# CristianSimion5/vk-raytracing-engine

Measured on AMD Instinct MI355X. Metric: Mrays/s, higher is better.
Workload: dtype f32

## Files before the change

vk-raytracing-engine_amd/csrc/shade.h:

```cpp
#pragma once
#include "device_math.h"
#include "device_scene.h"
#include "traverse.h"

struct Payload
{
  f3 hitValue;
  uint32_t seed;
  uint32_t depth;
  f3 rayOrigin, rayDirection, weight;
  bool isSpecular;
  float lightDist;
  f3 shadowRayDir;
};

struct ShadeStats
{
  unsigned hits, diffuse, taps;
  const float* lut;
};

VKRT_DEV const float* ldsTexelLut(const DevScene& sc, float* lds512)
{
  for(unsigned i = threadIdx.x; i < 512u; i += blockDim.x)
// ... 277 lines not shown
{
  f3 worldPos, N, tangent, binormal, V, baseColor, emittance;
  float metalU, roughU;
  unsigned retap;
};

VKRT_DEV void closestHitFront(const DevScene& sc, const RayHit& hit, const uint32_t instId, const uint4 ts, f3 worldRayDir, const Payload& prd,
                              ShadeStats& st, HitMid& mid)
{
  st.hits++;
  const uint32_t i0 = ts.x, i1 = ts.y, i2 = ts.z, matIndex = ts.w;
  const f3 b = mk3(1.0f - hit.u - hit.v, hit.u, hit.v);

  const BufView vPN = bufView(sc.vertexPN), vMat = bufView(sc.shadeMaterials), vInst = bufView(sc.instances);
  const float4 a0 = bufLoad4(vPN, VKRT_VERTEX_BYTES * i0), b0 = bufLoad4(vPN, VKRT_VERTEX_BYTES * i0 + 16u), tq0 = bufLoad4(vPN, VKRT_VERTEX_BYTES * i0 + 32u);
  const float4 a1 = bufLoad4(vPN, VKRT_VERTEX_BYTES * i1), b1 = bufLoad4(vPN, VKRT_VERTEX_BYTES * i1 + 16u), tq1 = bufLoad4(vPN, VKRT_VERTEX_BYTES * i1 + 32u);
  const float4 a2 = bufLoad4(vPN, VKRT_VERTEX_BYTES * i2), b2 = bufLoad4(vPN, VKRT_VERTEX_BYTES * i2 + 16u), tq2 = bufLoad4(vPN, VKRT_VERTEX_BYTES * i2 + 32u);
  const uint32_t mo = 64u * matIndex;
  const float4 m0 = bufLoad4(vMat, mo), m1 = bufLoad4(vMat, mo + 16u), ref01 = bufLoad4(vMat, mo + 32u), ref23 = bufLoad4(vMat, mo + 48u);
  const uint32_t dimB = __float_as_uint(ref01.x), baseB = __float_as_uint(ref01.y), dimM = __float_as_uint(ref01.z), baseM = __float_as_uint(ref01.w);
  const uint32_t dimN = __float_as_uint(ref23.x), baseN = __float_as_uint(ref23.y), dimE = __float_as_uint(ref23.z), baseE = __float_as_uint(ref23.w);
  DevInstance in;
  {
    const uint32_t io = 96u * instId;
    const float4 q0 = bufLoad4(vInst, io), q1 = bufLoad4(vInst, io + 16u), q2 = bufLoad4(vInst, io + 32u), q3 = bufLoad4(vInst, io + 48u), q4 = bufLoad4(vInst, io + 64u),
                 q5 = bufLoad4(vInst, io + 80u);
    in.o2w[0] = q0.x; in.o2w[1] = q0.y; in.o2w[2] = q0.z; in.o2w[3] = q0.w; in.o2w[4] = q1.x; in.o2w[5] = q1.y; in.o2w[6] = q1.z; in.o2w[7] = q1.w;
    in.o2w[8] = q2.x; in.o2w[9] = q2.y; in.o2w[10] = q2.z; in.o2w[11] = q2.w;
    in.w2o[0] = q3.x; in.w2o[1] = q3.y; in.w2o[2] = q3.z; in.w2o[3] = q3.w; in.w2o[4] = q4.x; in.w2o[5] = q4.y; in.w2o[6] = q4.z; in.w2o[7] = q4.w;
    in.w2o[8] = q5.x; in.primMesh = __float_as_int(q5.y); in.vis = 0u; in.pad = 0;
  }
  GltfPBRMaterial mat;
  mat.pbrBaseColorFactor[0] = m0.x; mat.pbrBaseColorFactor[1] = m0.y; mat.pbrBaseColorFactor[2] = m0.z; mat.pbrBaseColorFactor[3] = 1.0f;
  mat.metallicFactor = m0.w; mat.roughnessFactor = m1.x;
  mat.emissiveFactor[0] = m1.y; mat.emissiveFactor[1] = m1.z; mat.emissiveFactor[2] = m1.w;
  mat.pbrBaseColorTexture = (dimB & 0x8000u) ? 0 : -1; mat.metallicRoughnessTexture = (dimM & 0x8000u) ? 0 : -1;
  mat.normalTexture = (dimN & 0x8000u) ? 0 : -1; mat.emissiveTexture = (dimE & 0x8000u) ? 0 : -1;
  const float tu = (b0.z * b.x + b1.z * b.y) + b2.z * b.z;
  const float tv = (b0.w * b.x + b1.w * b.y) + b2.w * b.z;

  const bool emits = prd.depth == 0 || prd.isSpecular;
  const bool wantE = emits && mat.emissiveTexture > -1, wantN = mat.normalTexture > -1;
  const bool wantB = mat.pbrBaseColorTexture > -1, wantM = mat.metallicRoughnessTexture > -1;
  st.taps += (wantE ? 1u : 0u) + (wantN ? 1u : 0u) + (wantB ? 1u : 0u) + (wantM ? 1u : 0u);
  TexTap tE, tN, tB, tM;
#define VKRT_FOOTPRINT(dim, base, want, tap)                                                                                           \
  texFootprint(sc.texQuads ? 0u : ((base) & 0x7fffffffu), ((dim) & 0x7fffu) + 1u, (((dim) >> 16) & 0x7fffu) + 1u, ((base) >> 31) != 0u, \
               ((dim) >> 31) != 0u, want, tu, tv, tap)
  VKRT_FOOTPRINT(dimE, baseE, wantE, tE);
  VKRT_FOOTPRINT(dimN, baseN, wantN, tN);
  VKRT_FOOTPRINT(dimB, baseB, wantB, tB);
  VKRT_FOOTPRINT(dimM, baseM, wantM, tM);
#undef VKRT_FOOTPRINT
  uint32_t e00, e10, e01, e11, n00, n10, n01, n11, c00, c10, c01, c11, r00, r10, r01, r11;
  if(sc.texQuads)
  {
    const BufView quads = bufView(sc.texQuads);
#define VKRT_QUAD(dim, base, tap, want, a, b, c, d)                                                                                    \
  {                                                                                                                                    \
    const uint32_t rec_ = ((want) && ((dim) >> 31) != 0u) ? tap.i00 + ((base) & 0x7fffffffu) : 0u;                                        \
    const float4 v_ = bufLoad4(quads, 16u * rec_);                                                                                     \
    a = __float_as_uint(v_.x); b = __float_as_uint(v_.y); c = __float_as_uint(v_.z); d = __float_as_uint(v_.w);                        \
  }
    VKRT_QUAD(dimE, baseE, tE, wantE, e00, e10, e01, e11)
    VKRT_QUAD(dimN, baseN, tN, wantN, n00, n10, n01, n11)
    VKRT_QUAD(dimB, baseB, tB, wantB, c00, c10, c01, c11)
    VKRT_QUAD(dimM, baseM, tM, wantM, r00, r10, r01, r11)
#undef VKRT_QUAD
  }
  else
  {
    const BufView tex = bufView(sc.texels);
#define VKRT_TEXEL(i) bufLoad1(tex, 4u * (i))
    e00 = VKRT_TEXEL(tE.i00); e10 = VKRT_TEXEL(tE.i10); e01 = VKRT_TEXEL(tE.i01); e11 = VKRT_TEXEL(tE.i11);
    n00 = VKRT_TEXEL(tN.i00); n10 = VKRT_TEXEL(tN.i10); n01 = VKRT_TEXEL(tN.i01); n11 = VKRT_TEXEL(tN.i11);
    c00 = VKRT_TEXEL(tB.i00); c10 = VKRT_TEXEL(tB.i10); c01 = VKRT_TEXEL(tB.i01); c11 = VKRT_TEXEL(tB.i11);
    r00 = VKRT_TEXEL(tM.i00); r10 = VKRT_TEXEL(tM.i10); r01 = VKRT_TEXEL(tM.i01); r11 = VKRT_TEXEL(tM.i11);
#undef VKRT_TEXEL
  }

  const f3 pos = mk3(a0.x, a0.y, a0.z) * b.x + mk3(a1.x, a1.y, a1.z) * b.y + mk3(a2.x, a2.y, a2.z) * b.z;
  const f3 worldPos = xformPoint(in, pos);
  const f3 nrm = normalize3(mk3(a0.w, b0.x, b0.y) * b.x + mk3(a1.w, b1.x, b1.y) * b.y + mk3(a2.w, b2.x, b2.y) * b.z);
  const f3 worldNrm = normalize3(xformNormal(in, nrm));
  const f3 tag = normalize3(mk3(tq0.x, tq0.y, tq0.z) * b.x + mk3(tq1.x, tq1.y, tq1.z) * b.y + mk3(tq2.x, tq2.y, tq2.z) * b.z);
  f3 worldTag = normalize3(xformNormal(in, tag));
  worldTag = normalize3(worldTag - dot3(worldTag, worldNrm) * worldNrm);
  const f3 worldBin = tq0.w * cross3(worldNrm, worldTag);

  f3 emittance = mk3(0.0f);
  if(emits)
  {
    emittance = mk3(mat.emissiveFactor[0], mat.emissiveFactor[1], mat.emissiveFactor[2]);
    if(wantE)
    {
      const f4 t = texBlend(st.lut, tE, e00, e10, e01, e11);
      emittance = emittance * mk3(t.x, t.y, t.z);
    }
  }
  f3 tangent = worldTag, binormal = worldBin;
  f3 texNormal = worldNrm;
  if(wantN)
  {
    const f4 t = texBlend(st.lut, tN, n00, n10, n01, n11);
    texNormal = normalize3(mk3(t.x, t.y, t.z) * 2.0f - mk3(1.0f));
    texNormal = normalize3(tangent * texNormal.x + binormal * texNormal.y + worldNrm * texNormal.z);
    createCoordinateSystem(texNormal, tangent, binormal);
  }
  f3 baseColor = mk3(mat.pbrBaseColorFactor[0], mat.pbrBaseColorFactor[1], mat.pbrBaseColorFactor[2]);
  if(wantB)
  {
    const f4 t = texBlend(st.lut, tB, c00, c10, c01, c11);
    baseColor = baseColor * mk3(t.x, t.y, t.z);
  }
  float metalness = mat.metallicFactor, roughness = mat.roughnessFactor;
  if(wantM)
  {
    const f4 t = texBlend(st.lut, tM, r00, r10, r01, r11);
    roughness *= t.y;
    metalness *= t.z;
  }

  mid.worldPos = worldPos; mid.N = texNormal; mid.tangent = tangent; mid.binormal = binormal;
  mid.V = normalize3(-worldRayDir);
  mid.baseColor = baseColor; mid.emittance = emittance;
  mid.metalU = metalness; mid.roughU = roughness;
  mid.retap = (mat.pbrBaseColorTexture > -1 ? 1u : 0u) + (mat.metallicRoughnessTexture > -1 ? 1u : 0u);
}

VKRT_DEV bool closestHitLobe(const HitMid& mid, Payload& prd)
// ... 105 lines not shown
```

vk-raytracing-engine_amd/csrc/wavefront.hip:

```cpp
#include <hip/hip_runtime.h>
#include <algorithm>
#include <cstdlib>
#include <cstring>

#include "device_math.h"
#include "device_scene.h"
#include "kernels.h"
#include "rgen.h"
#include "shade.h"
#include "traverse.h"
#include "traverse_wide.h"
#include "traverse_share.h"

#define WF_BLOCK 256
#define VKRT_FLAG_COUNT_WORK 2u

#include "wf_streams.h"

VKRT_DEV unsigned packFlags(const LaneState& L)
{
  return (L.prd.depth & 0xffu) | (((unsigned)L.smpl & 0xffffu) << 8) | ((L.prd.isSpecular ? 1u : 0u) << 25);
}

VKRT_DEV void loadCommon(const TraceParams& P, const WfBuffers& B, int parity, int type, unsigned i, LaneState& L)
{
  const float4 s0 = wfLoad(rec(B, parity, type, WF_S0, i)), s1 = wfLoad(rec(B, parity, type, WF_S1, i)), s2 = wfLoad(rec(B, parity, type, WF_S2, i));
  const unsigned flags = __float_as_uint(s1.w), pix = __float_as_uint(s2.w);
  L.curWeight = mk3(s0.x, s0.y, s0.z); L.prd.seed = __float_as_uint(s0.w);
  L.hitValue = mk3(s1.x, s1.y, s1.z);
  L.prd.depth = flags & 0xffu; L.smpl = (int)((flags >> 8) & 0xffffu);
  L.prd.isSpecular = ((flags >> 25) & 1u) != 0u;
  L.hitValues = mk3(s2.x, s2.y, s2.z);
  L.px = pix & 0xffffu; L.lrow = pix >> 16;
  float origin[4];
  mat4MulVec4(P.viewInverse, 0.0f, 0.0f, 0.0f, 1.0f, origin);
  L.camOrigin = mk3(origin[0], origin[1], origin[2]);
  L.prd.lightDist = 0.0f;
  L.prd.shadowRayDir = mk3(0.0f);
  L.prd.hitValue = mk3(0.0f);
  L.prd.weight = mk3(0.0f);
  L.stage = 0;
}

VKRT_DEV void storeState(const WfBuffers& B, int parity, int type, unsigned i, const LaneState& L, f3 weight)
{
  wfStore(rec(B, parity, type, WF_S0, i), make_float4(weight.x, weight.y, weight.z, __uint_as_float(L.prd.seed)));
  wfStore(rec(B, parity, type, WF_S1, i), make_float4(L.hitValue.x, L.hitValue.y, L.hitValue.z, __uint_as_float(packFlags(L))));
  wfStore(rec(B, parity, type, WF_S2, i), make_float4(L.hitValues.x, L.hitValues.y, L.hitValues.z, __uint_as_float(L.px | (L.lrow << 16))));
}

VKRT_DEV void storeClosest(const WfBuffers& B, int parity, unsigned i, const LaneState& L)
{
  wfStore(rec(B, parity, WF_C, WF_R0, i), make_float4(L.prd.rayOrigin.x, L.prd.rayOrigin.y, L.prd.rayOrigin.z, 10000.0f));
  wfStore(rec(B, parity, WF_C, WF_R1, i), make_float4(L.prd.rayDirection.x, L.prd.rayDirection.y, L.prd.rayDirection.z, 0.0f));
  storeState(B, parity, WF_C, i, L, L.curWeight);
}

VKRT_DEV void storeShadow(const WfBuffers& B, int parity, int type, unsigned i, const LaneState& L, f3 contrib, f3 nextWeight)
{
  wfStore(rec(B, parity, type, WF_R0, i), make_float4(L.prd.rayOrigin.x, L.prd.rayOrigin.y, L.prd.rayOrigin.z, L.prd.lightDist - 0.1f));
  wfStore(rec(B, parity, type, WF_R1, i), make_float4(L.prd.shadowRayDir.x, L.prd.shadowRayDir.y, L.prd.shadowRayDir.z, L.prd.lightDist));
  if(type == WF_P)
    wfStore(rec(B, parity, type, WF_R2, i), make_float4(L.prd.rayDirection.x, L.prd.rayDirection.y, L.prd.rayDirection.z, 0.0f));
  storeState(B, parity, type, i, L, nextWeight);
  wfStore(rec(B, parity, type, WF_S3, i), make_float4(contrib.x, contrib.y, contrib.z, 0.0f));
}

VKRT_DEV unsigned claimSlots(const WfBuffers& B, int parity, int to, unsigned lane, unsigned* wsum)
{
  const unsigned wave = threadIdx.x >> 6, nw = blockDim.x >> 6;
  const unsigned long long m[WF_TYPES] = {__ballot(to == WF_C), __ballot(to == WF_S), __ballot(to == WF_P)};
  if(lane == 0)
  {
#pragma unroll
    for(int t = 0; t < WF_TYPES; t++) wsum[t * (nw + 1) + wave] = (unsigned)__popcll(m[t]);
  }
  __syncthreads();
  if(threadIdx.x < WF_TYPES)
  {
    unsigned* w = wsum + threadIdx.x * (nw + 1);
    unsigned tot = 0;
    for(unsigned k = 0; k < nw; k++)
    {
      const unsigned c = w[k];
      w[k] = tot;
      tot += c;
    }
    w[nw] = tot ? atomicAdd(countOf(B, parity, (int)threadIdx.x), tot) : 0u;
  }
  __syncthreads();
  if(to < 0)
    return 0u;
  const unsigned long long below = (1ull << lane) - 1ull;
  const unsigned long long mine = to == WF_C ? m[0] : to == WF_S ? m[1] : m[2];
  return wsum[to * (nw + 1) + nw] + wsum[to * (nw + 1) + wave] + (unsigned)__popcll(mine & below);
}

__global__ __launch_bounds__(WF_BLOCK) void k_wf_init(const TraceParams P, const WfBuffers B)
{
  const unsigned lane = lane_id();
  const unsigned w = blockIdx.x * blockDim.x + threadIdx.x;
  bool alive = false;
  unsigned nPixels = 0;
  LaneState L;
  if(w < P.tileCount * 64u)
  {
    const unsigned tile = P.tileFirst + (w >> 6), inTile = w & 63u;
    const uint32_t x = (tile % P.tilesX) * 8u + (inTile & 7u);
    const uint32_t lrow = (tile / P.tilesX) * 8u + (inTile >> 3);
    if(x < P.fullW && lrow < P.localRows)
    {
      const uint32_t y = globalRow(P, lrow);
      if(y < P.fullH)
      {
        startPixel(P, L, x, y, lrow);
        nPixels = 1;
        if(P.pc.samples <= 0 || P.pc.depth <= 0)
          storePixel(P, L);
        else
          alive = true;
      }
    }
  }
  __shared__ unsigned wsum[WF_TYPES * (WF_BLOCK / 64 + 1)];
  const unsigned slot = claimSlots(B, 0, alive ? WF_C : -1, lane, wsum);
  if(alive)
    storeClosest(B, 0, slot, L);
  __shared__ unsigned long long red[VKRT_COUNTER_STRIDE * (WF_BLOCK / 64)];
  const unsigned vals[6] = {0, 0, 0, 0, 0, nPixels};
  blockAddCounters(&P.counters->v[blockIdx.x % VKRT_COUNTER_SLOTS][0], vals, 6, red);
}

VKRT_DEV void hybridFinish(const TraceParams& P, const HybridGi& G, uint32_t px, uint32_t lrow, bool shaded, f3 hitValue, float hitDists, float alpha)
{
  const size_t p = (size_t)lrow * P.fullW + px;
  float4 color = make_float4(0.0f, 0.0f, 0.0f, alpha);
  if(shaded)
  {
    color.x = hitValue.x; color.y = hitValue.y; color.z = hitValue.z;
    if(G.nrdRadHitD)
    {
      const float roughness = G.rough[p].x;
      const float viewZ = G.nrdViewZ[p];
      const float t = glsl_clamp(exp2f(-25.0f * roughness * roughness), 0.0f, 1.0f);
      const float f = (3.0f + fabsf(viewZ) * 1.0f) * (1.0f * (1.0f - t) + 20.0f * t);
      float normHitDist = glsl_clamp(hitDists / f, 0.0f, 1.0f);
      f3 rad = hitValue;
      const bool bad = isnan(rad.x) || isnan(rad.y) || isnan(rad.z) || isinf(rad.x) || isinf(rad.y) || isinf(rad.z);
      rad = bad ? mk3(0.0f) : mk3(glsl_clamp(rad.x, 0.0f, 65504.0f), glsl_clamp(rad.y, 0.0f, 65504.0f), glsl_clamp(rad.z, 0.0f, 65504.0f));
      normHitDist = (isnan(normHitDist) || isinf(normHitDist)) ? 0.0f : glsl_clamp(normHitDist, 0.0f, 1.0f);
      if(normHitDist != 0.0f)
        normHitDist = glsl_max(normHitDist, 1e-7f);
      const float Y = (rad.x * 0.25f + rad.y * 0.5f) + rad.z * 0.25f;
      const float Co = (rad.x * 0.5f + rad.y * 0.0f) + rad.z * -0.5f;
      const float Cg = (rad.x * -0.25f + rad.y * 0.5f) + rad.z * -0.25f;
      G.nrdRadHitD[p] = make_float4(quantizeHalf(Y), quantizeHalf(Co), quantizeHalf(Cg), quantizeHalf(normHitDist));
    }
  }
  if(P.pc.frame > 0)
  {
    const float a = 1.0f / (float)(P.pc.frame + 1);
    const float4 old = G.accum[p];
    G.accum[p] = make_float4(old.x * (1.0f - a) + color.x * a, old.y * (1.0f - a) + color.y * a, old.z * (1.0f - a) + color.z * a,
                             old.w * (1.0f - a) + color.w * a);
  }
  else
    G.accum[p] = color;
}
VKRT_DEV bool advanceSegmentHybrid(const TraceParams& P, const HybridGi& G, LaneState& L, bool shadowHit, f3 contrib, f3 nextWeight, float lightDist)
{
  L.stage = 0;
  if(!shadowHit)
    L.hitValue = L.hitValue + contrib;
  if(L.prd.depth == 1u && !L.prd.isSpecular)
    L.hitValues.x = shadowHit ? 0.5f * lightDist : lightDist;
  L.curWeight = nextWeight;
  L.prd.depth++;
  if(!(L.prd.depth < (uint32_t)P.pc.depth))
  {
    hybridFinish(P, G, L.px, L.lrow, true, L.hitValue, L.hitValues.x, L.hitValues.y);
    return false;
  }
  return true;
}

struct ShadeLds
{
  float lut[512];
  unsigned wsum[WF_TYPES * (WF_BLOCK / 64 + 1)];
};

template <bool PAIR, bool HYBRID>
VKRT_DEV void shadeHitBlock(const TraceParams& P, const WfBuffers& B, const HybridGi& G, const int par, const unsigned count, const unsigned block, ShadeLds& lds)
{
  const int type = PAIR ? WF_P : WF_C;
  const unsigned lane = lane_id();
  const unsigned qi = block * WF_BLOCK + threadIdx.x;
  ShadeStats st;
  st.hits = 0; st.diffuse = 0; st.taps = 0;
  st.lut = ldsTexelLut(P.sc, lds.lut);
  unsigned* wsum = lds.wsum;
  int to = -1;
  LaneState L;
  f3 contrib = mk3(0.0f), nextWeight = mk3(0.0f);
  if(qi < count)
  {
    loadCommon(P, B, par, type, qi, L);
    const float4 h = wfLoad(rec(B, par, type, WF_H0, qi)), t4 = wfLoad(rec(B, par, type, WF_H1, qi));
    const float4 rd = wfLoad(rec(B, par, type, PAIR ? WF_R2 : WF_R1, qi));
    L.prd.rayDirection = mk3(rd.x, rd.y, rd.z);
    L.prd.rayOrigin = mk3(0.0f);
    if(PAIR)
    {
      const float4 s3 = wfLoad(rec(B, par, WF_P, WF_S3, qi));
      const bool shadowHit = __float_as_int(h.x) != 0;
      if(HYBRID)
        (void)advanceSegmentHybrid(P, G, L, shadowHit, mk3(s3.x, s3.y, s3.z), L.curWeight, L.prd.depth == 1u ? wfLoad(rec(B, par, WF_P, WF_R1, qi)).w : 0.0f);
      else
        (void)advanceSegment(P, L, shadowHit, mk3(s3.x, s3.y, s3.z), L.curWeight);
    }
    RayHit hit;
    hit.t = h.x; hit.u = h.y; hit.v = h.z; hit.slot = __float_as_int(h.w);
    const uint4 ts = make_uint4(__float_as_uint(t4.x), __float_as_uint(t4.y), __float_as_uint(t4.z), __float_as_uint(t4.w));
    if(hit.slot >= 0)
      closestHitShaderInst(P.sc, P.pc, hit, (uint32_t)hit.slot, ts, L.prd.rayDirection, L.prd, st);
    else
      missShader(P.pc, L.prd);
    segmentTerms(L, contrib, nextWeight);
    const bool dead = !HYBRID && (P.flags & VKRT_FLAG_SKIP_DEAD_SHADOW) != 0u && contrib.x == 0.0f && contrib.y == 0.0f && contrib.z == 0.0f;
    if(!L.prd.isSpecular && L.prd.depth != 100u && !dead)
      to = (L.prd.depth + 1u < (uint32_t)P.pc.depth) ? WF_P : WF_S;
    else if(HYBRID)
      to = advanceSegmentHybrid(P, G, L, false, contrib, nextWeight, 0.0f) ? WF_C : -1;
    else
      to = advanceSegment(P, L, false, contrib, nextWeight) ? WF_C : -1;
  }
  const unsigned slot = claimSlots(B, par ^ 1, to, lane, wsum);
  if(to == WF_C)
    storeClosest(B, par ^ 1, slot, L);
  else if(to >= 0)
    storeShadow(B, par ^ 1, to, slot, L, contrib, nextWeight);
  if(P.flags & VKRT_FLAG_COUNT_WORK)
  {
    __shared__ unsigned long long red[VKRT_COUNTER_STRIDE * (WF_BLOCK / 64)];
    const unsigned vals[5] = {0, 0, st.hits, st.diffuse, st.taps};
    blockAddCounters(&P.counters->v[blockIdx.x % VKRT_COUNTER_SLOTS][0], vals, 5, red);
  }
}

template <bool HYBRID>
VKRT_DEV void shadeShadowBlock(const TraceParams& P, const WfBuffers& B, const HybridGi& G, const int par, const unsigned count, const unsigned block, ShadeLds& lds)
{
  const unsigned lane = lane_id();
  const unsigned qi = block * WF_BLOCK + threadIdx.x;
  unsigned* wsum = lds.wsum;
  bool toClosest = false;
  LaneState L;
  if(qi < count)
  {
    loadCommon(P, B, par, WF_S, qi, L);
    const float4 h = wfLoad(rec(B, par, WF_S, WF_H0, qi)), s3 = wfLoad(rec(B, par, WF_S, WF_S3, qi));
    L.prd.rayOrigin = mk3(0.0f);
    L.prd.rayDirection = mk3(0.0f);
    const bool shadowHit = __float_as_int(h.w) >= 0;
    if(HYBRID)
      toClosest = advanceSegmentHybrid(P, G, L, shadowHit, mk3(s3.x, s3.y, s3.z), L.curWeight, L.prd.depth == 1u ? wfLoad(rec(B, par, WF_S, WF_R1, qi)).w : 0.0f);
    else
      toClosest = advanceSegment(P, L, shadowHit, mk3(s3.x, s3.y, s3.z), L.curWeight);
  }
  const unsigned slot = claimSlots(B, par ^ 1, toClosest ? WF_C : -1, lane, wsum);
  if(toClosest)
    storeClosest(B, par ^ 1, slot, L);
}

template <bool HYBRID>
VKRT_DEV void shadeRound(const TraceParams& P, const WfBuffers& B, const HybridGi& G, const int round)
{
  const int par = round & 1;
  const unsigned cC = *countOf(B, par, WF_C), cS = *countOf(B, par, WF_S), cP = *countOf(B, par, WF_P);
  const unsigned nC = (cC + WF_BLOCK - 1) / WF_BLOCK, nP = (cP + WF_BLOCK - 1) / WF_BLOCK, nS = (cS + WF_BLOCK - 1) / WF_BLOCK;
  unsigned blk = blockIdx.x;
  __shared__ ShadeLds lds;
  if(blk < nC)
    shadeHitBlock<false, HYBRID>(P, B, G, par, cC, blk, lds);
  else if((blk -= nC) < nP)
    shadeHitBlock<true, HYBRID>(P, B, G, par, cP, blk, lds);
  else if((blk -= nP) < nS)
    shadeShadowBlock<HYBRID>(P, B, G, par, cS, blk, lds);
}
__global__ __launch_bounds__(WF_BLOCK) void k_wf_shade(const TraceParams P, const WfBuffers B, const int round)
{
  const HybridGi none{};
  shadeRound<false>(P, B, none, round);
}
__global__ __launch_bounds__(WF_BLOCK) void k_wf_shade_hybrid(const TraceParams P, const WfBuffers B, const HybridGi G, const int round)
{
  shadeRound<true>(P, B, G, round);
}

__global__ __launch_bounds__(WF_BLOCK) void k_hy_gi_init(const TraceParams P, const WfBuffers B, const HybridGi G, const uint2* tmp)
{
  const unsigned lane = lane_id();
  const unsigned w = blockIdx.x * blockDim.x + threadIdx.x;
  bool alive = false;
  LaneState L;
  if(w < P.tileCount * 64u)
  {
    const unsigned tile = P.tileFirst + (w >> 6), inTile = w & 63u;
    const uint32_t x = (tile % P.tilesX) * 8u + (inTile & 7u);
    const uint32_t lrow = (tile / P.tilesX) * 8u + (inTile >> 3);
    if(x < P.fullW && lrow < P.localRows && globalRow(P, lrow) < P.fullH)
    {
      const size_t p = (size_t)lrow * P.fullW + x;
      const float4 pixelImg = G.color[p], pixelPos = G.position[p], pixelNorm = G.normal[p];
      const float2 rm = G.rough[p];
      const uint2 t = tmp[p];
      const f3 worldPos = mk3(pixelPos.x, pixelPos.y, pixelPos.z), worldNrm = mk3(pixelNorm.x, pixelNorm.y, pixelNorm.z);
      const bool shaded = !(worldPos.x == 0.0f && worldPos.y == 0.0f && worldPos.z == 0.0f && worldNrm.x == 0.0f && worldNrm.y == 0.0f &&
                            worldNrm.z == 0.0f);
      const float alpha = __uint_as_float(t.y);
      if(!shaded)
        hybridFinish(P, G, x, lrow, false, mk3(0.0f), 0.0f, alpha);
      else
      {
        L.px = x; L.lrow = lrow;
        L.prd.seed = t.x;
        L.prd.lightDist = 0.0f; L.prd.shadowRayDir = mk3(0.0f);
        const float roughness = rm.x, metalness = rm.y;
        const float ratio = metalness * (1.0f - roughness);
        f3 direction;
        if(ratio < 0.8f)
        {
          L.prd.isSpecular = false;
          f3 tangent, binormal;
          createCoordinateSystem(worldNrm, tangent, binormal);
          direction = normalize3(samplingHemisphere(L.prd.seed, tangent, binormal, worldNrm));
          L.curWeight = mk3(pixelImg.w, pixelPos.w, pixelNorm.w);
        }
        else
        {
          L.prd.isSpecular = true;
          float cam[4];
          mat4MulVec4(P.viewInverse, 0.0f, 0.0f, 0.0f, 1.0f, cam);
          const f3 V = normalize3(mk3(cam[0], cam[1], cam[2]) - worldPos);
          direction = normalize3(glsl_reflect(-V, worldNrm));
          L.curWeight = mk3(1.0f);
        }
        L.prd.hitValue = mk3(0.0f);
        L.prd.rayOrigin = worldPos;
        L.prd.rayDirection = direction;
        L.prd.depth = 1;
        L.prd.weight = mk3(0.0f);
        L.hitValue = mk3(0.0f);
        L.hitValues = mk3(0.0f, alpha, 0.0f);
        L.smpl = 0;
        L.stage = 0;
        if(L.prd.depth < (uint32_t)P.pc.depth)
          alive = true;
        else
          hybridFinish(P, G, x, lrow, true, mk3(0.0f), 0.0f, alpha);
      }
    }
  }
  __shared__ unsigned wsum[WF_TYPES * (WF_BLOCK / 64 + 1)];
  const unsigned slot = claimSlots(B, 0, alive ? WF_C : -1, lane, wsum);
  if(alive)
    storeClosest(B, 0, slot, L);
}

__global__ __launch_bounds__(WF_BLOCK) void k_wf_blend(const TraceParams P, const float4* stage)
{
  const unsigned w = blockIdx.x * blockDim.x + threadIdx.x;
  if(w >= P.tileCount * 64u)
    return;
  const unsigned tile = P.tileFirst + (w >> 6), inTile = w & 63u;
  const uint32_t x = (tile % P.tilesX) * 8u + (inTile & 7u);
  const uint32_t lrow = (tile / P.tilesX) * 8u + (inTile >> 3);
  if(x < P.fullW && lrow < P.localRows && globalRow(P, lrow) < P.fullH)
  {
    const size_t p = (size_t)lrow * P.fullW + x;
    blendPixel((float4*)P.image + p, stage[p], P.pc.frame);
  }
}

#define WF_CTRL_BYTES (256 * VKRT_WF_MAX_LANES)
size_t vkrt_wf_state_bytes(uint32_t pathCapacity, int groups)
{
  const size_t g = (size_t)std::max(groups, 1);
  return g * pathCapacity * 2 * WF_SLOTS * sizeof(float4) + (g > 1 ? g * pathCapacity * sizeof(float4) : 0) + WF_CTRL_BYTES;
}

void vkrt_wf_carve(void* base, uint32_t pathCapacity, int groups, WfBuffers* B)
{
  const size_t g = (size_t)std::max(groups, 1);
  char* p = (char*)base;
  B->ctrl = (unsigned*)p;
  p += WF_CTRL_BYTES;
  B->planes = (float4*)p;
  p += g * pathCapacity * 2 * WF_SLOTS * sizeof(float4);
  B->stage = g > 1 ? (float4*)p : nullptr;
  B->capacity = pathCapacity;
  B->groups = (uint32_t)g;
}

static hipError_t subframeBegin(const TraceParams& P, const WfBuffers& B, hipStream_t stream)
{
  const unsigned work = P.tileCount * 64u;
  const hipError_t e = hipMemsetAsync(B.ctrl, 0, 64, stream);
  if(e != hipSuccess)
    return e;
  hipLaunchKernelGGL(k_wf_init, dim3((work + WF_BLOCK - 1) / WF_BLOCK), dim3(WF_BLOCK), 0, stream, P, B);
  return hipSuccess;
}
static int subframeRounds(const TraceParams& P) { return (P.pc.samples <= 0 || P.pc.depth <= 0) ? 0 : P.pc.samples * (P.pc.depth + 1); }
static void subframeRound(const TraceParams& P, const WfBuffers& B, int r, unsigned travBlock, bool count, hipStream_t stream, WfTiming* timing)
{
  const unsigned work = P.tileCount * 64u;
  const dim3 tg(2 * ((work + travBlock - 1) / travBlock) + 4);
  const size_t tlds = (size_t)P.sc.stackCap * travBlock * sizeof(int);
  const bool timed = timing && timing->events && 2 * (timing->used + 1) <= timing->capacity;
  if(timed)
    (void)hipEventRecord(timing->events[2 * timing->used], stream);
  vkrt_wf_launch_traverse(P, B, r, travBlock, count, tg, tlds, stream);
  if(timed)
  {
    (void)hipEventRecord(timing->events[2 * timing->used + 1], stream);
    timing->used++;
  }
  hipLaunchKernelGGL(k_wf_shade, dim3((work + WF_BLOCK - 1) / WF_BLOCK + 3), dim3(WF_BLOCK), 0, stream, P, B, r);
}

static TraceParams frameParams(const TraceParams& P, int k, uint32_t seedStep)
{
  TraceParams Q = P;
  Q.pc.frame = P.pc.frame + k;
  Q.seed = P.seed + (uint32_t)k * seedStep;
  return Q;
}

static int balancedInFlight(int frames, int want)
{
  want = std::max(1, std::min(want, frames));
  const int turns = (frames + want - 1) / want;
  return (frames + turns - 1) / turns;
}

hipError_t vkrt_launch_wavefront(const TraceParams& P, const WfBuffers& B, const WfOptions& opt, int frames, uint32_t seedStep, bool count,
                                 hipStream_t stream, WfTiming* timing, const WfAsync* async)
{
  const unsigned travBlock = opt.travBlock == 256 ? 256u : opt.travBlock == 128 ? 128u : 64u;
  const int rounds = subframeRounds(P);
  frames = std::max(frames, 1);
  int F = (timing || !async || rounds == 0) ? 1 : std::min(balancedInFlight(frames, opt.inFlight), (int)B.groups);
  F = std::max(1, std::min(F, async ? std::min(VKRT_WF_MAX_LANES, async->count) : 1));
  int S = (timing || !async || F > 1) ? 1 : std::max(1, std::min(std::min(VKRT_WF_MAX_LANES, opt.subframes), async->count));
  S = (int)std::min<uint32_t>((uint32_t)S, std::max(1u, P.tileCount / 256u));
  const int L = S * F;
  hipError_t e;
  if(L <= 1)
  {
    for(int k = 0; k < frames; k++)
    {
      TraceParams Q = frameParams(P, k, seedStep);
      Q.tileFirst = 0;
      if((e = subframeBegin(Q, B, stream)) != hipSuccess) return e;
      for(int r = 0; r < rounds; r++) subframeRound(Q, B, r, travBlock, count, stream, timing);
    }
    return hipGetLastError();
  }
  const bool staged = F > 1;
  if(staged && vkrt_wf_pool_events(frames, S) > async->poolSize)
    return hipErrorInvalidValue;
  hipStream_t laneStream[VKRT_WF_MAX_LANES];
  uint32_t tile0[VKRT_WF_MAX_LANES], tileN[VKRT_WF_MAX_LANES];
  WfBuffers Bq[VKRT_WF_MAX_LANES];
  const size_t groupQuads = (size_t)2 * WF_SLOTS * B.capacity;
  for(int q = 0; q < L; q++)
  {
    const int g = q / S, j = q % S;
    tile0[q] = (uint32_t)((uint64_t)P.tileCount * j / S);
    tileN[q] = (uint32_t)((uint64_t)P.tileCount * (j + 1) / S) - tile0[q];
    Bq[q].ctrl = B.ctrl + 64 * q;
    Bq[q].planes = B.planes + (size_t)g * groupQuads + (size_t)2 * WF_SLOTS * ((size_t)tile0[q] * 64u);
    Bq[q].stage = staged ? B.stage + (size_t)g * B.capacity : nullptr;
    Bq[q].capacity = tileN[q] * 64u;
    Bq[q].groups = 1;
    laneStream[q] = async->streams[q];
  }
  int forked = 0;
  auto joinLanes = [&]() {
    hipError_t first = hipSuccess;
    for(int q = 0; q < forked; q++)
    {
      hipError_t x = hipEventRecord(async->join[q], laneStream[q]);
      if(x == hipSuccess) x = hipStreamWaitEvent(stream, async->join[q], 0);
      if(x != hipSuccess)
      {
        (void)hipStreamSynchronize(laneStream[q]);
        if(first == hipSuccess) first = x;
      }
    }
    return first;
  };
  if((e = hipEventRecord(async->fork, stream)) != hipSuccess) return e;
  for(int q = 0; q < L; q++)
  {
    if((e = hipStreamWaitEvent(laneStream[q], async->fork, 0)) != hipSuccess)
    {
      (void)joinLanes();
      return e;
    }
    forked = q + 1;
  }
  const int items = rounds + 1 + (staged ? 1 : 0);
  hipEvent_t* evBlend = async->pool;
  int laneFrames[VKRT_WF_MAX_LANES], cursor[VKRT_WF_MAX_LANES];
  std::vector<char> blendRecorded(staged ? (size_t)frames * S : 0, 0);
  int remaining = 0;
  for(int q = 0; q < L; q++)
  {
    laneFrames[q] = (frames - q / S + F - 1) / F;
    cursor[q] = 0;
    remaining += laneFrames[q] * items;
  }
  e = hipSuccess;
  while(remaining > 0 && e == hipSuccess)
  {
    bool progressed = false;
    for(int q = 0; q < L && e == hipSuccess; q++)
    {
      if(cursor[q] >= laneFrames[q] * items)
        continue;
      const int g = q / S, j = q % S, m = cursor[q] / items, it = cursor[q] % items, k = g + m * F;
      TraceParams Q = frameParams(P, k, seedStep);
      Q.tileFirst = tile0[q];
      Q.tileCount = tileN[q];
      if(staged)
// ... 64 lines not shown
```

vk-raytracing-engine_amd/csrc/wf_streams.h:

```cpp
#pragma once
#include <hip/hip_runtime.h>

#include "device_math.h"
#include "device_scene.h"
#include "traverse_wide.h"

#define WF_PLANES 9
#define WF_TYPES 3
enum { WF_R0 = 0, WF_R1, WF_R2, WF_H0, WF_H1, WF_S0, WF_S1, WF_S2, WF_S3 };
enum { WF_C = 0, WF_S = 1, WF_P = 2 };

#define WF_SLOTS_CS 8
#define WF_SLOTS (WF_SLOTS_CS + WF_PLANES)
VKRT_DEV float4* plane(const WfBuffers& B, int parity, int type, int k)
{
  const int slot = type == WF_P ? WF_SLOTS_CS + k : (k > WF_R2 ? k - 1 : k);
  return B.planes + ((size_t)(parity * WF_SLOTS + slot)) * B.capacity;
}
VKRT_DEV unsigned* countOf(const WfBuffers& B, int parity, int type) { return &B.ctrl[parity * 4 + type]; }
VKRT_DEV float4* rec(const WfBuffers& B, int parity, int type, int k, unsigned i)
{
  return (float4*)((char*)plane(B, parity, type, k) + (size_t)((type == WF_S ? B.capacity - 1u - i : i) * 16u));
}

VKRT_DEV float4 wfLoad(const float4* p)
{
  const vkrt_v4f v = __builtin_nontemporal_load((const vkrt_v4f*)p);
  return make_float4(v.x, v.y, v.z, v.w);
}
VKRT_DEV void wfStore(float4* p, float4 v) { *p = v; }
```

vk-raytracing-engine_amd/csrc/wf_traverse.hip:

```cpp
#include <hip/hip_runtime.h>

#include "device_math.h"
#include "device_scene.h"
#include "kernels.h"
#include "traverse.h"
#include "traverse_wide.h"
#include "traverse_share.h"
#include "wf_streams.h"

enum { WF_K_CLOSEST_C = 0, WF_K_CLOSEST_P = 1, WF_K_SHADOW_S = 2, WF_K_SHADOW_P = 3 };

VKRT_DEV void storeHit(const TraceParams& P, const WfBuffers& B, int par, int kind, unsigned qi, const RayHit& hit)
{
  if(kind == WF_K_SHADOW_S)
    wfStore(rec(B, par, WF_S, WF_H0, qi), make_float4(0.0f, 0.0f, 0.0f, __int_as_float(hit.slot >= 0 ? 0 : -1)));
  else if(kind == WF_K_SHADOW_P)
    ((float*)rec(B, par, WF_P, WF_H0, qi))[0] = __int_as_float(hit.slot >= 0 ? 1 : 0);
  else
  {
    const int type = kind == WF_K_CLOSEST_C ? WF_C : WF_P;
    int inst = -1;
    if(hit.slot >= 0)
    {
      const uint4 ts = P.sc.triShade[hit.slot];
      inst = __float_as_int(P.sc.tris[hit.slot * VKRT_TRI_QUADS + 2].z);
      wfStore(rec(B, par, type, WF_H1, qi), make_float4(__uint_as_float(ts.x), __uint_as_float(ts.y), __uint_as_float(ts.z), __uint_as_float(ts.w)));
    }
    float* h = (float*)rec(B, par, type, WF_H0, qi);
    if(type == WF_C)
      wfStore(rec(B, par, WF_C, WF_H0, qi), make_float4(hit.t, hit.u, hit.v, __int_as_float(inst)));
    else
    {
      h[1] = hit.u; h[2] = hit.v; h[3] = __int_as_float(inst);
    }
  }
}

template <bool COUNT, bool WIDE, int TB, int TM = 0>
__global__ __launch_bounds__(TB)
__attribute__((amdgpu_waves_per_eu(TM != 0 && WIDE && TB == 64 ? 5 : 1)))
void k_wf_traverse(const TraceParams P, const WfBuffers B, const int round)
{
  extern __shared__ int lds_stack[];
  const int par = round & 1;
  const unsigned cC = *countOf(B, par, WF_C), cS = *countOf(B, par, WF_S), cP = *countOf(B, par, WF_P);
  if(blockIdx.x == 0 && threadIdx.x == 0)
  {
    for(int t = 0; t < WF_TYPES; t++) *countOf(B, par ^ 1, t) = 0u;
    if(cC + cP) atomicAdd(&P.counters->v[round % VKRT_COUNTER_SLOTS][0], (unsigned long long)cC + cP);
    if(cS + cP) atomicAdd(&P.counters->v[round % VKRT_COUNTER_SLOTS][1], (unsigned long long)cS + cP);
    if(cP) atomicAdd(&P.counters->v[round % VKRT_COUNTER_SLOTS][11], (unsigned long long)cP);
  }
  const unsigned nC = (cC + TB - 1) / TB, nP = (cP + TB - 1) / TB, nS = (cS + TB - 1) / TB;
  unsigned blk = blockIdx.x;
  int kind;
  unsigned count;
  if(blk < nC) { kind = WF_K_CLOSEST_C; count = cC; }
  else if((blk -= nC) < nP) { kind = WF_K_CLOSEST_P; count = cP; }
  else if((blk -= nP) < nS) { kind = WF_K_SHADOW_S; count = cS; }
  else if((blk -= nS) < nP) { kind = WF_K_SHADOW_P; count = cP; }
  else return;
  const bool anyHit = kind >= WF_K_SHADOW_S;
  const int type = kind == WF_K_CLOSEST_C ? WF_C : kind == WF_K_SHADOW_S ? WF_S : WF_P;
  const unsigned qi = blk * TB + threadIdx.x;
  const bool valid = qi < count;
  float4 r0 = make_float4(0.0f, 0.0f, 0.0f, 0.0f), r1 = make_float4(1.0f, 0.0f, 0.0f, 0.0f);
  if(valid)
  {
// ... 64 lines not shown
```

Measured before the change: 4994.

## Shrink wavefront path state and skip dead texture fetches

Non-hybrid paths no longer carry the S2 state record. The pixel word now rides in spare lanes of R1/S3, and accumulated radiance goes to a per-pixel stage buffer that is read and written only when a path ends. Shadow hit flags become single-word stores and loads, and texture quad and texel loads are guarded so absent textures are never fetched. This cuts global memory traffic per path segment in exchange for scattered per-pixel stage accesses and extra branches in shading.

```diff
diff --git a/vk-raytracing-engine_amd/csrc/shade.h b/vk-raytracing-engine_amd/csrc/shade.h
--- a/vk-raytracing-engine_amd/csrc/shade.h
+++ b/vk-raytracing-engine_amd/csrc/shade.h
@@ -353,30 +353,33 @@
   VKRT_FOOTPRINT(dimB, baseB, wantB, tB);
   VKRT_FOOTPRINT(dimM, baseM, wantM, tM);
 #undef VKRT_FOOTPRINT
-  uint32_t e00, e10, e01, e11, n00, n10, n01, n11, c00, c10, c01, c11, r00, r10, r01, r11;
+  uint32_t e00 = 0u, e10 = 0u, e01 = 0u, e11 = 0u, n00 = 0u, n10 = 0u, n01 = 0u, n11 = 0u, c00 = 0u, c10 = 0u, c01 = 0u, c11 = 0u, r00 = 0u, r10 = 0u,
+           r01 = 0u, r11 = 0u;
+  const bool liveE = wantE && (dimE >> 31) != 0u, liveN = wantN && (dimN >> 31) != 0u, liveB = wantB && (dimB >> 31) != 0u,
+             liveM = wantM && (dimM >> 31) != 0u;
   if(sc.texQuads)
   {
     const BufView quads = bufView(sc.texQuads);
-#define VKRT_QUAD(dim, base, tap, want, a, b, c, d)                                                                                    \
+#define VKRT_QUAD(base, tap, live, a, b, c, d)                                                                                         \
+  if(live)                                                                                                                             \
   {                                                                                                                                    \
-    const uint32_t rec_ = ((want) && ((dim) >> 31) != 0u) ? tap.i00 + ((base) & 0x7fffffffu) : 0u;                                        \
-    const float4 v_ = bufLoad4(quads, 16u * rec_);                                                                                     \
+    const float4 v_ = bufLoad4(quads, 16u * (tap.i00 + ((base) & 0x7fffffffu)));                                                       \
     a = __float_as_uint(v_.x); b = __float_as_uint(v_.y); c = __float_as_uint(v_.z); d = __float_as_uint(v_.w);                        \
   }
-    VKRT_QUAD(dimE, baseE, tE, wantE, e00, e10, e01, e11)
-    VKRT_QUAD(dimN, baseN, tN, wantN, n00, n10, n01, n11)
-    VKRT_QUAD(dimB, baseB, tB, wantB, c00, c10, c01, c11)
-    VKRT_QUAD(dimM, baseM, tM, wantM, r00, r10, r01, r11)
+    VKRT_QUAD(baseE, tE, liveE, e00, e10, e01, e11)
+    VKRT_QUAD(baseN, tN, liveN, n00, n10, n01, n11)
+    VKRT_QUAD(baseB, tB, liveB, c00, c10, c01, c11)
+    VKRT_QUAD(baseM, tM, liveM, r00, r10, r01, r11)
 #undef VKRT_QUAD
   }
   else
   {
     const BufView tex = bufView(sc.texels);
 #define VKRT_TEXEL(i) bufLoad1(tex, 4u * (i))
-    e00 = VKRT_TEXEL(tE.i00); e10 = VKRT_TEXEL(tE.i10); e01 = VKRT_TEXEL(tE.i01); e11 = VKRT_TEXEL(tE.i11);
-    n00 = VKRT_TEXEL(tN.i00); n10 = VKRT_TEXEL(tN.i10); n01 = VKRT_TEXEL(tN.i01); n11 = VKRT_TEXEL(tN.i11);
-    c00 = VKRT_TEXEL(tB.i00); c10 = VKRT_TEXEL(tB.i10); c01 = VKRT_TEXEL(tB.i01); c11 = VKRT_TEXEL(tB.i11);
-    r00 = VKRT_TEXEL(tM.i00); r10 = VKRT_TEXEL(tM.i10); r01 = VKRT_TEXEL(tM.i01); r11 = VKRT_TEXEL(tM.i11);
+    if(liveE) { e00 = VKRT_TEXEL(tE.i00); e10 = VKRT_TEXEL(tE.i10); e01 = VKRT_TEXEL(tE.i01); e11 = VKRT_TEXEL(tE.i11); }
+    if(liveN) { n00 = VKRT_TEXEL(tN.i00); n10 = VKRT_TEXEL(tN.i10); n01 = VKRT_TEXEL(tN.i01); n11 = VKRT_TEXEL(tN.i11); }
+    if(liveB) { c00 = VKRT_TEXEL(tB.i00); c10 = VKRT_TEXEL(tB.i10); c01 = VKRT_TEXEL(tB.i01); c11 = VKRT_TEXEL(tB.i11); }
+    if(liveM) { r00 = VKRT_TEXEL(tM.i00); r10 = VKRT_TEXEL(tM.i10); r01 = VKRT_TEXEL(tM.i01); r11 = VKRT_TEXEL(tM.i11); }
 #undef VKRT_TEXEL
   }
 
diff --git a/vk-raytracing-engine_amd/csrc/wavefront.hip b/vk-raytracing-engine_amd/csrc/wavefront.hip
--- a/vk-raytracing-engine_amd/csrc/wavefront.hip
+++ b/vk-raytracing-engine_amd/csrc/wavefront.hip
@@ -22,10 +22,12 @@
   return (L.prd.depth & 0xffu) | (((unsigned)L.smpl & 0xffffu) << 8) | ((L.prd.isSpecular ? 1u : 0u) << 25);
 }
 
-VKRT_DEV void loadCommon(const TraceParams& P, const WfBuffers& B, int parity, int type, unsigned i, LaneState& L)
-{
-  const float4 s0 = wfLoad(rec(B, parity, type, WF_S0, i)), s1 = wfLoad(rec(B, parity, type, WF_S1, i)), s2 = wfLoad(rec(B, parity, type, WF_S2, i));
-  const unsigned flags = __float_as_uint(s1.w), pix = __float_as_uint(s2.w);
+template <bool HYBRID>
+VKRT_DEV void loadCommon(const TraceParams& P, const WfBuffers& B, int parity, int type, unsigned i, unsigned pix, LaneState& L)
+{
+  const float4 s0 = wfLoad(rec(B, parity, type, WF_S0, i)), s1 = wfLoad(rec(B, parity, type, WF_S1, i));
+  const float4 s2 = HYBRID ? wfLoad(rec(B, parity, type, WF_S2, i)) : make_float4(0.0f, 0.0f, 0.0f, 0.0f);
+  const unsigned flags = __float_as_uint(s1.w);
   L.curWeight = mk3(s0.x, s0.y, s0.z); L.prd.seed = __float_as_uint(s0.w);
   L.hitValue = mk3(s1.x, s1.y, s1.z);
   L.prd.depth = flags & 0xffu; L.smpl = (int)((flags >> 8) & 0xffffu);
@@ -42,28 +44,49 @@
   L.stage = 0;
 }
 
+VKRT_DEV float pixelWord(const LaneState& L) { return __uint_as_float(L.px | (L.lrow << 16)); }
+
+template <bool HYBRID>
 VKRT_DEV void storeState(const WfBuffers& B, int parity, int type, unsigned i, const LaneState& L, f3 weight)
 {
   wfStore(rec(B, parity, type, WF_S0, i), make_float4(weight.x, weight.y, weight.z, __uint_as_float(L.prd.seed)));
   wfStore(rec(B, parity, type, WF_S1, i), make_float4(L.hitValue.x, L.hitValue.y, L.hitValue.z, __uint_as_float(packFlags(L))));
-  wfStore(rec(B, parity, type, WF_S2, i), make_float4(L.hitValues.x, L.hitValues.y, L.hitValues.z, __uint_as_float(L.px | (L.lrow << 16))));
-}
-
+  if(HYBRID)
+    wfStore(rec(B, parity, type, WF_S2, i), make_float4(L.hitValues.x, L.hitValues.y, L.hitValues.z, 0.0f));
+}
+
+template <bool HYBRID>
 VKRT_DEV void storeClosest(const WfBuffers& B, int parity, unsigned i, const LaneState& L)
 {
   wfStore(rec(B, parity, WF_C, WF_R0, i), make_float4(L.prd.rayOrigin.x, L.prd.rayOrigin.y, L.prd.rayOrigin.z, 10000.0f));
-  wfStore(rec(B, parity, WF_C, WF_R1, i), make_float4(L.prd.rayDirection.x, L.prd.rayDirection.y, L.prd.rayDirection.z, 0.0f));
-  storeState(B, parity, WF_C, i, L, L.curWeight);
-}
-
+  wfStore(rec(B, parity, WF_C, WF_R1, i), make_float4(L.prd.rayDirection.x, L.prd.rayDirection.y, L.prd.rayDirection.z, pixelWord(L)));
+  storeState<HYBRID>(B, parity, WF_C, i, L, L.curWeight);
+}
+
+template <bool HYBRID>
 VKRT_DEV void storeShadow(const WfBuffers& B, int parity, int type, unsigned i, const LaneState& L, f3 contrib, f3 nextWeight)
 {
   wfStore(rec(B, parity, type, WF_R0, i), make_float4(L.prd.rayOrigin.x, L.prd.rayOrigin.y, L.prd.rayOrigin.z, L.prd.lightDist - 0.1f));
   wfStore(rec(B, parity, type, WF_R1, i), make_float4(L.prd.shadowRayDir.x, L.prd.shadowRayDir.y, L.prd.shadowRayDir.z, L.prd.lightDist));
   if(type == WF_P)
     wfStore(rec(B, parity, type, WF_R2, i), make_float4(L.prd.rayDirection.x, L.prd.rayDirection.y, L.prd.rayDirection.z, 0.0f));
-  storeState(B, parity, type, i, L, nextWeight);
-  wfStore(rec(B, parity, type, WF_S3, i), make_float4(contrib.x, contrib.y, contrib.z, 0.0f));
+  storeState<HYBRID>(B, parity, type, i, L, nextWeight);
+  wfStore(rec(B, parity, type, WF_S3, i), make_float4(contrib.x, contrib.y, contrib.z, pixelWord(L)));
+}
+
+VKRT_DEV bool advanceSegmentSum(const TraceParams& P, const WfBuffers& B, LaneState& L, bool shadowHit, f3 contrib, f3 nextWeight)
+{
+  const bool ends = !(L.prd.depth + 1u < (uint32_t)P.pc.depth);
+  float4* sum = B.stage + ((size_t)L.lrow * P.fullW + L.px);
+  if(ends)
+  {
+    const float4 v = *sum;
+    L.hitValues = mk3(v.x, v.y, v.z);
+  }
+  const bool on = advanceSegment(P, L, shadowHit, contrib, nextWeight);
+  if(ends && on)
+    *sum = make_float4(L.hitValues.x, L.hitValues.y, L.hitValues.z, 0.0f);
+  return on;
 }
 
 VKRT_DEV unsigned claimSlots(const WfBuffers& B, int parity, int to, unsigned lane, unsigned* wsum)
@@ -125,7 +148,10 @@
   __shared__ unsigned wsum[WF_TYPES * (WF_BLOCK / 64 + 1)];
   const unsigned slot = claimSlots(B, 0, alive ? WF_C : -1, lane, wsum);
   if(alive)
-    storeClosest(B, 0, slot, L);
+  {
+    B.stage[(size_t)L.lrow * P.fullW + L.px] = make_float4(0.0f, 0.0f, 0.0f, 0.0f);
+    storeClosest<false>(B, 0, slot, L);
+  }
   __shared__ unsigned long long red[VKRT_COUNTER_STRIDE * (WF_BLOCK / 64)];
   const unsigned vals[6] = {0, 0, 0, 0, 0, nPixels};
   blockAddCounters(&P.counters->v[blockIdx.x % VKRT_COUNTER_SLOTS][0], vals, 6, red);
@@ -205,14 +231,16 @@
   f3 contrib = mk3(0.0f), nextWeight = mk3(0.0f);
   if(qi < count)
   {
-    loadCommon(P, B, par, type, qi, L);
     const float4 h = wfLoad(rec(B, par, type, WF_H0, qi)), t4 = wfLoad(rec(B, par, type, WF_H1, qi));
     const float4 rd = wfLoad(rec(B, par, type, PAIR ? WF_R2 : WF_R1, qi));
+    float4 s3 = make_float4(0.0f, 0.0f, 0.0f, 0.0f);
+    if(PAIR)
+      s3 = wfLoad(rec(B, par, WF_P, WF_S3, qi));
+    loadCommon<HYBRID>(P, B, par, type, qi, __float_as_uint(PAIR ? s3.w : rd.w), L);
     L.prd.rayDirection = mk3(rd.x, rd.y, rd.z);
     L.prd.rayOrigin = mk3(0.0f);
     if(PAIR)
     {
-      const float4 s3 = wfLoad(rec(B, par, WF_P, WF_S3, qi));
       const bool shadowHit = __float_as_int(h.x) != 0;
       if(HYBRID)
         (void)advanceSegmentHybrid(P, G, L, shadowHit, mk3(s3.x, s3.y, s3.z), L.curWeight, L.prd.depth == 1u ? wfLoad(rec(B, par, WF_P, WF_R1, qi)).w : 0.0f);
@@ -233,13 +261,13 @@
     else if(HYBRID)
       to = advanceSegmentHybrid(P, G, L, false, contrib, nextWeight, 0.0f) ? WF_C : -1;
     else
-      to = advanceSegment(P, L, false, contrib, nextWeight) ? WF_C : -1;
+      to = advanceSegmentSum(P, B, L, false, contrib, nextWeight) ? WF_C : -1;
   }
   const unsigned slot = claimSlots(B, par ^ 1, to, lane, wsum);
   if(to == WF_C)
-    storeClosest(B, par ^ 1, slot, L);
+    storeClosest<HYBRID>(B, par ^ 1, slot, L);
   else if(to >= 0)
-    storeShadow(B, par ^ 1, to, slot, L, contrib, nextWeight);
+    storeShadow<HYBRID>(B, par ^ 1, to, slot, L, contrib, nextWeight);
   if(P.flags & VKRT_FLAG_COUNT_WORK)
   {
     __shared__ unsigned long long red[VKRT_COUNTER_STRIDE * (WF_BLOCK / 64)];
@@ -258,19 +286,20 @@
   LaneState L;
   if(qi < count)
   {
-    loadCommon(P, B, par, WF_S, qi, L);
-    const float4 h = wfLoad(rec(B, par, WF_S, WF_H0, qi)), s3 = wfLoad(rec(B, par, WF_S, WF_S3, qi));
+    const float4 s3 = wfLoad(rec(B, par, WF_S, WF_S3, qi));
+    const float occluded = wfLoad1((const float*)rec(B, par, WF_S, WF_H0, qi) + 3);
+    loadCommon<HYBRID>(P, B, par, WF_S, qi, __float_as_uint(s3.w), L);
     L.prd.rayOrigin = mk3(0.0f);
     L.prd.rayDirection = mk3(0.0f);
-    const bool shadowHit = __float_as_int(h.w) >= 0;
+    const bool shadowHit = __float_as_int(occluded) >= 0;
     if(HYBRID)
       toClosest = advanceSegmentHybrid(P, G, L, shadowHit, mk3(s3.x, s3.y, s3.z), L.curWeight, L.prd.depth == 1u ? wfLoad(rec(B, par, WF_S, WF_R1, qi)).w : 0.0f);
     else
-      toClosest = advanceSegment(P, L, shadowHit, mk3(s3.x, s3.y, s3.z), L.curWeight);
+      toClosest = advanceSegmentSum(P, B, L, shadowHit, mk3(s3.x, s3.y, s3.z), L.curWeight);
   }
   const unsigned slot = claimSlots(B, par ^ 1, toClosest ? WF_C : -1, lane, wsum);
   if(toClosest)
-    storeClosest(B, par ^ 1, slot, L);
+    storeClosest<HYBRID>(B, par ^ 1, slot, L);
 }
 
 template <bool HYBRID>
@@ -365,7 +394,7 @@
   __shared__ unsigned wsum[WF_TYPES * (WF_BLOCK / 64 + 1)];
   const unsigned slot = claimSlots(B, 0, alive ? WF_C : -1, lane, wsum);
   if(alive)
-    storeClosest(B, 0, slot, L);
+    storeClosest<true>(B, 0, slot, L);
 }
 
 __global__ __launch_bounds__(WF_BLOCK) void k_wf_blend(const TraceParams P, const float4* stage)
@@ -387,7 +416,7 @@
 size_t vkrt_wf_state_bytes(uint32_t pathCapacity, int groups)
 {
   const size_t g = (size_t)std::max(groups, 1);
-  return g * pathCapacity * 2 * WF_SLOTS * sizeof(float4) + (g > 1 ? g * pathCapacity * sizeof(float4) : 0) + WF_CTRL_BYTES;
+  return g * pathCapacity * 2 * WF_SLOTS * sizeof(float4) + g * pathCapacity * sizeof(float4) + WF_CTRL_BYTES;
 }
 
 void vkrt_wf_carve(void* base, uint32_t pathCapacity, int groups, WfBuffers* B)
@@ -398,7 +427,7 @@
   p += WF_CTRL_BYTES;
   B->planes = (float4*)p;
   p += g * pathCapacity * 2 * WF_SLOTS * sizeof(float4);
-  B->stage = g > 1 ? (float4*)p : nullptr;
+  B->stage = (float4*)p;
   B->capacity = pathCapacity;
   B->groups = (uint32_t)g;
 }
@@ -482,7 +511,7 @@
     tileN[q] = (uint32_t)((uint64_t)P.tileCount * (j + 1) / S) - tile0[q];
     Bq[q].ctrl = B.ctrl + 64 * q;
     Bq[q].planes = B.planes + (size_t)g * groupQuads + (size_t)2 * WF_SLOTS * ((size_t)tile0[q] * 64u);
-    Bq[q].stage = staged ? B.stage + (size_t)g * B.capacity : nullptr;
+    Bq[q].stage = B.stage + (size_t)g * B.capacity;
     Bq[q].capacity = tileN[q] * 64u;
     Bq[q].groups = 1;
     laneStream[q] = async->streams[q];
diff --git a/vk-raytracing-engine_amd/csrc/wf_streams.h b/vk-raytracing-engine_amd/csrc/wf_streams.h
--- a/vk-raytracing-engine_amd/csrc/wf_streams.h
+++ b/vk-raytracing-engine_amd/csrc/wf_streams.h
@@ -28,4 +28,5 @@
   const vkrt_v4f v = __builtin_nontemporal_load((const vkrt_v4f*)p);
   return make_float4(v.x, v.y, v.z, v.w);
 }
+VKRT_DEV float wfLoad1(const float* p) { return __builtin_nontemporal_load(p); }
 VKRT_DEV void wfStore(float4* p, float4 v) { *p = v; }
diff --git a/vk-raytracing-engine_amd/csrc/wf_traverse.hip b/vk-raytracing-engine_amd/csrc/wf_traverse.hip
--- a/vk-raytracing-engine_amd/csrc/wf_traverse.hip
+++ b/vk-raytracing-engine_amd/csrc/wf_traverse.hip
@@ -13,7 +13,7 @@
 VKRT_DEV void storeHit(const TraceParams& P, const WfBuffers& B, int par, int kind, unsigned qi, const RayHit& hit)
 {
   if(kind == WF_K_SHADOW_S)
-    wfStore(rec(B, par, WF_S, WF_H0, qi), make_float4(0.0f, 0.0f, 0.0f, __int_as_float(hit.slot >= 0 ? 0 : -1)));
+    ((float*)rec(B, par, WF_S, WF_H0, qi))[3] = __int_as_float(hit.slot >= 0 ? 0 : -1);
   else if(kind == WF_K_SHADOW_P)
     ((float*)rec(B, par, WF_P, WF_H0, qi))[0] = __int_as_float(hit.slot >= 0 ? 1 : 0);
   else
```

Result: slower. 4930 (-1.3%).

## Regroup shading lanes by BRDF lobe through LDS to reduce wave divergence

Applied to the files above, without the earlier changes.

The closest-hit shader is split into a front part (surface interpolation) and a tail part (lobe-specific BRDF sampling). Between the two, every thread in the block is permuted through LDS so that diffuse hits, specular hits and misses form contiguous groups, using per-wave ballots and a block prefix sum. The aim is to cut SIMD divergence in the tail shading. The cost is extra block barriers, roughly 36 floats per thread of LDS traffic, and a larger LDS footprint that may lower occupancy.

```diff
diff --git a/vk-raytracing-engine_amd/csrc/wavefront.hip b/vk-raytracing-engine_amd/csrc/wavefront.hip
--- a/vk-raytracing-engine_amd/csrc/wavefront.hip
+++ b/vk-raytracing-engine_amd/csrc/wavefront.hip
@@ -184,11 +184,95 @@
   return true;
 }
 
+#define WF_XCHG_QUADS 9
+#define WF_XCHG_PASSES 1
+#define WF_XCHG_PASS_QUADS ((WF_XCHG_QUADS + WF_XCHG_PASSES - 1) / WF_XCHG_PASSES)
 struct ShadeLds
 {
   float lut[512];
   unsigned wsum[WF_TYPES * (WF_BLOCK / 64 + 1)];
+  unsigned lobes[2 * (WF_BLOCK / 64)];
+  float4 xchg[WF_BLOCK][WF_XCHG_PASS_QUADS];
 };
+
+VKRT_DEV void regroupByLobe(ShadeLds& lds, const unsigned lane, const unsigned nValid, bool& valid, bool& hit, bool& diffuse, HitMid& mid, LaneState& L)
+{
+  const unsigned wave = threadIdx.x >> 6, nw = WF_BLOCK / 64;
+  const bool isD = hit && diffuse, isS = hit && !diffuse;
+  const unsigned long long mD = __ballot(isD), mS = __ballot(isS);
+  if(lane == 0)
+  {
+    lds.lobes[wave] = (unsigned)__popcll(mD);
+    lds.lobes[nw + wave] = (unsigned)__popcll(mS);
+  }
+  __syncthreads();
+  unsigned nD = 0, nS = 0, dBelow = 0, sBelow = 0;
+#pragma unroll
+  for(unsigned k = 0; k < nw; k++)
+  {
+    const unsigned d = lds.lobes[k], s = lds.lobes[nw + k];
+    dBelow += k < wave ? d : 0u; sBelow += k < wave ? s : 0u;
+    nD += d; nS += s;
+  }
+  const unsigned long long below = (1ull << lane) - 1ull;
+  const unsigned rD = dBelow + (unsigned)__popcll(mD & below), rS = sBelow + (unsigned)__popcll(mS & below);
+  const unsigned dest = isD ? rD : isS ? WF_BLOCK - nS + rS : nD + (threadIdx.x - rD - rS);
+  const bool home = valid;
+  float4 q[WF_XCHG_QUADS];
+  if(home)
+  {
+    q[0] = make_float4(mid.worldPos.x, mid.worldPos.y, mid.worldPos.z, mid.metalU);
+    q[1] = make_float4(mid.N.x, mid.N.y, mid.N.z, mid.roughU);
+    q[2] = make_float4(mid.tangent.x, mid.tangent.y, mid.tangent.z, __uint_as_float(mid.retap));
+    q[3] = make_float4(mid.binormal.x, mid.binormal.y, mid.binormal.z, __uint_as_float(L.prd.seed));
+    q[4] = make_float4(mid.V.x, mid.V.y, mid.V.z, __uint_as_float(packFlags(L)));
+    q[5] = make_float4(mid.baseColor.x, mid.baseColor.y, mid.baseColor.z, __uint_as_float(L.px | (L.lrow << 16)));
+    q[6] = make_float4(mid.emittance.x, mid.emittance.y, mid.emittance.z, L.curWeight.x);
+    q[7] = make_float4(L.curWeight.y, L.curWeight.z, L.hitValue.x, L.hitValue.y);
+    q[8] = make_float4(L.hitValue.z, L.hitValues.x, L.hitValues.y, L.hitValues.z);
+  }
+  diffuse = threadIdx.x < nD;
+  hit = diffuse || threadIdx.x >= WF_BLOCK - nS;
+  valid = hit || threadIdx.x < nValid - nS;
+#pragma unroll
+  for(int p = 0; p < WF_XCHG_PASSES; p++)
+  {
+    if(p > 0)
+      __syncthreads();
+    if(home)
+    {
+#pragma unroll
+      for(int k = 0; k < WF_XCHG_PASS_QUADS; k++)
+        if(p * WF_XCHG_PASS_QUADS + k < WF_XCHG_QUADS)
+          lds.xchg[dest][k] = q[p * WF_XCHG_PASS_QUADS + k];
+    }
+    __syncthreads();
+    if(valid)
+    {
+#pragma unroll
+      for(int k = 0; k < WF_XCHG_PASS_QUADS; k++)
+        if(p * WF_XCHG_PASS_QUADS + k < WF_XCHG_QUADS)
+          q[p * WF_XCHG_PASS_QUADS + k] = lds.xchg[threadIdx.x][k];
+    }
+  }
+  if(valid)
+  {
+    const float4 q0 = q[0], q1 = q[1], q2 = q[2], q3 = q[3], q4 = q[4], q5 = q[5], q6 = q[6], q7 = q[7], q8 = q[8];
+    mid.worldPos = mk3(q0.x, q0.y, q0.z); mid.metalU = q0.w;
+    mid.N = mk3(q1.x, q1.y, q1.z); mid.roughU = q1.w;
+    mid.tangent = mk3(q2.x, q2.y, q2.z); mid.retap = __float_as_uint(q2.w);
+    mid.binormal = mk3(q3.x, q3.y, q3.z); L.prd.seed = __float_as_uint(q3.w);
+    mid.V = mk3(q4.x, q4.y, q4.z);
+    const unsigned flags = __float_as_uint(q4.w), pix = __float_as_uint(q5.w);
+    L.prd.depth = flags & 0xffu; L.smpl = (int)((flags >> 8) & 0xffffu);
+    L.prd.isSpecular = ((flags >> 25) & 1u) != 0u;
+    mid.baseColor = mk3(q5.x, q5.y, q5.z); L.px = pix & 0xffffu; L.lrow = pix >> 16;
+    mid.emittance = mk3(q6.x, q6.y, q6.z);
+    L.curWeight = mk3(q6.w, q7.x, q7.y);
+    L.hitValue = mk3(q7.z, q7.w, q8.x);
+    L.hitValues = mk3(q8.y, q8.z, q8.w);
+  }
+}
 
 template <bool PAIR, bool HYBRID>
 VKRT_DEV void shadeHitBlock(const TraceParams& P, const WfBuffers& B, const HybridGi& G, const int par, const unsigned count, const unsigned block, ShadeLds& lds)
@@ -203,13 +287,14 @@
   int to = -1;
   LaneState L;
   f3 contrib = mk3(0.0f), nextWeight = mk3(0.0f);
-  if(qi < count)
+  HitMid mid = {};
+  bool valid = qi < count, hit = false, diffuse = false;
+  if(valid)
   {
     loadCommon(P, B, par, type, qi, L);
     const float4 h = wfLoad(rec(B, par, type, WF_H0, qi)), t4 = wfLoad(rec(B, par, type, WF_H1, qi));
     const float4 rd = wfLoad(rec(B, par, type, PAIR ? WF_R2 : WF_R1, qi));
     L.prd.rayDirection = mk3(rd.x, rd.y, rd.z);
-    L.prd.rayOrigin = mk3(0.0f);
     if(PAIR)
     {
       const float4 s3 = wfLoad(rec(B, par, WF_P, WF_S3, qi));
@@ -219,11 +304,31 @@
       else
         (void)advanceSegment(P, L, shadowHit, mk3(s3.x, s3.y, s3.z), L.curWeight);
     }
-    RayHit hit;
-    hit.t = h.x; hit.u = h.y; hit.v = h.z; hit.slot = __float_as_int(h.w);
+    RayHit hit_;
+    hit_.t = h.x; hit_.u = h.y; hit_.v = h.z; hit_.slot = __float_as_int(h.w);
     const uint4 ts = make_uint4(__float_as_uint(t4.x), __float_as_uint(t4.y), __float_as_uint(t4.z), __float_as_uint(t4.w));
-    if(hit.slot >= 0)
-      closestHitShaderInst(P.sc, P.pc, hit, (uint32_t)hit.slot, ts, L.prd.rayDirection, L.prd, st);
+    hit = hit_.slot >= 0;
+    if(hit)
+    {
+      closestHitFront(P.sc, hit_, (uint32_t)hit_.slot, ts, L.prd.rayDirection, L.prd, st, mid);
+      diffuse = closestHitLobe(mid, L.prd);
+    }
+  }
+  regroupByLobe(lds, lane, min(count - block * WF_BLOCK, (unsigned)WF_BLOCK), valid, hit, diffuse, mid, L);
+  if(valid)
+  {
+    float origin[4];
+    mat4MulVec4(P.viewInverse, 0.0f, 0.0f, 0.0f, 1.0f, origin);
+    L.camOrigin = mk3(origin[0], origin[1], origin[2]);
+    L.prd.lightDist = 0.0f;
+    L.prd.shadowRayDir = mk3(0.0f);
+    L.prd.hitValue = mk3(0.0f);
+    L.prd.weight = mk3(0.0f);
+    L.stage = 0;
+    L.prd.rayOrigin = mk3(0.0f);
+    L.prd.rayDirection = mk3(0.0f);
+    if(hit)
+      closestHitTail(P.sc, P.pc, mid, diffuse, L.prd, st);
     else
       missShader(P.pc, L.prd);
     segmentTerms(L, contrib, nextWeight);
```

Measured after the change: 5015 before, 4992 after. No clear change (-0.5%).
